# shadygm/Lichtfeld-Densification-Plugin

Measured on AMD Instinct MI355X. Metric: triangulated points/sec + pairs/sec, MipNeRF360 garden @fast, 1/2/4/8 GPU, higher is better.
Workload: dtype f32 (+f64 Sampson/DLT solve)

## Files before the change

lichtfeld-densification-plugin_amd/csrc/lfd_kernels.hip:

```cpp
#include <hip/hip_runtime.h>
#include <stdint.h>

#include "lfd_device.hpp"

namespace {

constexpr int kBlock = LFD_DENSE_BLOCK;
constexpr int kCpt = LFD_DENSE_CPT;
constexpr int kTile = kBlock * kCpt;

typedef unsigned long long u64;

constexpr u64 kStEmpty = 0ull, kStAggregate = 1ull, kStPrefix = 2ull;
constexpr u64 kValueMask = (1ull << LFD_VALUE_BITS) - 1ull;
__device__ __forceinline__ u64 pack_state(u64 st, unsigned epoch, u64 v) {
    return (st << 62) | ((u64)epoch << LFD_VALUE_BITS) | (v & kValueMask);
}
__device__ __forceinline__ u64 state_status(u64 s, unsigned epoch) {
    return (((s >> LFD_VALUE_BITS) & LFD_EPOCH_MASK) == epoch) ? (s >> 62) : kStEmpty;
}

__device__ __forceinline__ void state_store(u64* p, u64 v) {
    __hip_atomic_store(p, v, __ATOMIC_RELAXED, __HIP_MEMORY_SCOPE_AGENT);
}
// ... 178 lines not shown
    if (r >= W) { ++q; r -= W; }
    if (r < 0) { --q; r += W; }
    if (r >= W) { ++q; r -= W; }
    y = q; x = r;
}

__device__ __forceinline__ void lfd_divmod_local(int local, int W, float inv_w, int w_log2, int& dy, int& x) {
    if (w_log2 >= 0) { dy = local >> w_log2; x = local & (W - 1); return; }
    int q = (int)((float)local * inv_w);
    int r = local - __mul24(q, W);
    if (r < 0) { --q; r += W; }
    if (r >= W) { ++q; r -= W; }
    dy = q; x = r;
}

__device__ __forceinline__ float cell_cert(const LfdLaunch& L, const BlockShared& S, int j, int cell, int x, int y,
                                           float raw, float mask_a_val) {
    float c = lfd_cert_floor(raw, L.kp.certainty_thresh);
    if (S.ref.mask_a) c = c * mask_a_val;
    const uint8_t* mb = S.slot[j].mask_b;
    if (mb) {
        const float2 wv = load_f32x2(S.slot[j].warp + (size_t)cell * L.warp_channels + (L.warp_channels - 2));
        const int ix = lfd_grid_nearest(wv.x, L.W);
        const int iy = lfd_grid_nearest(wv.y, L.H);
        float m = 0.0f;
        if (ix >= 0 && iy >= 0)
            m = (float)lfd_global(mb)[(size_t)lfd_nearest_src(iy, L.mask_sy, L.h_match) * L.w_match + lfd_nearest_src(ix, L.mask_sx, L.w_match)];
        c = c * m;
    }
    return c;
}

__device__ __forceinline__ float cell_mask_a(const LfdLaunch& L, const BlockShared& S, int x, int y) {
    if (!S.ref.mask_a) return 1.0f;
    return (float)lfd_global(S.ref.mask_a)[(size_t)lfd_nearest_src(y, L.mask_sy, L.h_match) * L.w_match + lfd_nearest_src(x, L.mask_sx, L.w_match)];
}

__device__ __forceinline__ void argmax_step(float c, int j, float& best, int& bj) {
    const bool take = (c > best) || ((c != c) && !(best != best));
    if (take) { best = c; bj = j; }
}

__device__ __forceinline__ void cell_best(const LfdLaunch& L, const BlockShared& S, int cell, float& best, int& bj) {
    int y, x;
    lfd_divmod(cell, L.W, L.inv_w, y, x);
    const float ma = cell_mask_a(L, S, x, y);
    const int ns = S.ref.n_slots;
    best = cell_cert(L, S, 0, cell, x, y, lfd_global(S.slot[0].cert)[cell], ma);
    bj = 0;
    for (int j = 1; j < ns; ++j) argmax_step(cell_cert(L, S, j, cell, x, y, lfd_global(S.slot[j].cert)[cell], ma), j, best, bj);
}

__device__ __forceinline__ void cells4_best_masked(const LfdLaunch& L, const BlockShared& S, int cell0, int y, int x0,
                                                   float best[4], int bj[4]) {
    const float th = L.kp.certainty_thresh;
    float ma[4] = {1.0f, 1.0f, 1.0f, 1.0f};
    const bool has_a = S.ref.mask_a != nullptr;
    if (has_a) {
        const uint8_t LFD_GLOBAL_AS* row = lfd_global(S.ref.mask_a) + (size_t)lfd_nearest_src(y, L.mask_sy, L.h_match) * L.w_match;
#pragma unroll
        for (int e = 0; e < 4; ++e) ma[e] = (float)row[lfd_nearest_src(x0 + e, L.mask_sx, L.w_match)];
    }
    const int ns = S.ref.n_slots;
    for (int j = 0; j < ns; ++j) {
        const float4 c4 = load_f32x4(S.slot[j].cert + cell0);
        float c[4] = {lfd_cert_floor(c4.x, th), lfd_cert_floor(c4.y, th), lfd_cert_floor(c4.z, th), lfd_cert_floor(c4.w, th)};
        if (has_a) {
#pragma unroll
            for (int e = 0; e < 4; ++e) c[e] = c[e] * ma[e];
        }
        const uint8_t* mb = S.slot[j].mask_b;
        if (mb) {
            float wx[4], wy[4];
            const float* wp = S.slot[j].warp;
            if (L.warp_channels == 4) {
#pragma unroll
                for (int e = 0; e < 4; ++e) { const float4 v = load_f32x4(wp + (size_t)(unsigned)(cell0 + e) * 4); wx[e] = v.z; wy[e] = v.w; }
            } else {
                const float4 a = load_f32x4(wp + (size_t)(unsigned)cell0 * 2), b = load_f32x4(wp + (size_t)(unsigned)cell0 * 2 + 4);
                wx[0] = a.x; wy[0] = a.y; wx[1] = a.z; wy[1] = a.w; wx[2] = b.x; wy[2] = b.y; wx[3] = b.z; wy[3] = b.w;
            }
#pragma unroll
            for (int e = 0; e < 4; ++e) {
                const int ix = lfd_grid_nearest(wx[e], L.W);
                const int iy = lfd_grid_nearest(wy[e], L.H);
                float m = 0.0f;
                if (ix >= 0 && iy >= 0)
                    m = (float)lfd_global(mb)[(size_t)lfd_nearest_src(iy, L.mask_sy, L.h_match) * L.w_match + lfd_nearest_src(ix, L.mask_sx, L.w_match)];
                c[e] = c[e] * m;
            }
        }
        if (j == 0) {
#pragma unroll
            for (int e = 0; e < 4; ++e) { best[e] = c[e]; bj[e] = 0; }
        } else {
#pragma unroll
            for (int e = 0; e < 4; ++e) argmax_step(c[e], j, best[e], bj[e]);
        }
    }
}

__device__ __forceinline__ void cell_coords(const LfdLaunch& L, const BlockShared& S, int cell, int bj, float& xan,
                                            float& yan, float& xbn, float& ybn) {
    const float* wp = S.slot[bj].warp;
    if (L.warp_channels == 4) {
        const float4 v = load_f32x4(wp + (size_t)cell * 4);
        xan = v.x; yan = v.y; xbn = v.z; ybn = v.w;
    } else {
        const float2 v = load_f32x2(wp + (size_t)cell * 2);
        int y, x;
        lfd_divmod(cell, L.W, L.inv_w, y, x);
        xan = lfd_global(L.axis_x)[x]; yan = lfd_global(L.axis_y)[y];
        xbn = v.x; ybn = v.y;
    }
}

}

extern "C" __global__ void lfd_pair_setup_kernel(LfdLaunch L, LfdRefConst* __restrict__ ref_out,
                                                 LfdPairConst* __restrict__ pair_out) {
    const int i = (int)(blockIdx.x * blockDim.x + threadIdx.x);
    const int n_pairs = L.n_refs * L.k;
    if (i < n_pairs) {
        const int r = i / L.k, j = i - r * L.k;
        if (j < L.refs[r].n_slots) {
            lfd_make_pair_const(L.cams[L.refs[r].cam], L.cams[L.slots[i].cam], L.slots[i].cam, L.w_match, L.h_match, pair_out[i],
                                L.fund_override ? L.fund_override + (size_t)i * 9 : nullptr);
        }
    } else if (i < n_pairs + L.n_refs) {
        const int r = i - n_pairs;
        lfd_make_ref_const(L.cams[L.refs[r].cam], L.w_match, L.h_match, ref_out[r]);
    }
}

extern "C" __global__ void __launch_bounds__(256) lfd_aggregate_kernel(LfdLaunch L, float* __restrict__ best_cert,
                                                                       uint8_t* __restrict__ best_slot) {
    __shared__ BlockShared S;
    const int r = (int)blockIdx.y;
    const int tid = (int)threadIdx.x;
    if (tid == 0) S.ref = L.refs[r];
    if (tid < L.k) S.slot[tid] = L.slots[(size_t)r * L.k + tid];
    __syncthreads();
    const int HW = L.H * L.W;
    const bool plain = !S.ref.mask_a && (HW & 3) == 0;
    bool any_mask_b = false;
    for (int j = 0; j < S.ref.n_slots; ++j) any_mask_b |= (S.slot[j].mask_b != nullptr);
    const int ns = S.ref.n_slots;
    for (int base = ((int)blockIdx.x * 256 + tid) * 4; base < HW; base += (int)gridDim.x * 256 * 4) {
        if (plain && !any_mask_b && base + 3 < HW) {
            float4 best = load_f32x4(S.slot[0].cert + base);
            const float th = L.kp.certainty_thresh;
            best.x = lfd_cert_floor(best.x, th); best.y = lfd_cert_floor(best.y, th);
            best.z = lfd_cert_floor(best.z, th); best.w = lfd_cert_floor(best.w, th);
            int b0 = 0, b1 = 0, b2 = 0, b3 = 0;
            for (int j = 1; j < ns; ++j) {
                const float4 c = load_f32x4(S.slot[j].cert + base);
                argmax_step(lfd_cert_floor(c.x, th), j, best.x, b0);
                argmax_step(lfd_cert_floor(c.y, th), j, best.y, b1);
                argmax_step(lfd_cert_floor(c.z, th), j, best.z, b2);
                argmax_step(lfd_cert_floor(c.w, th), j, best.w, b3);
            }
            *reinterpret_cast<float4*>(best_cert + (size_t)r * HW + base) = best;
            if (best_slot) {
                const unsigned packed = (unsigned)b0 | ((unsigned)b1 << 8) | ((unsigned)b2 << 16) | ((unsigned)b3 << 24);
                *reinterpret_cast<unsigned*>(best_slot + (size_t)r * HW + base) = packed;
            }
        } else if ((L.W & 3) == 0 && (HW & 3) == 0 && base + 3 < HW) {
            int y, x0;
            lfd_divmod(base, L.W, L.inv_w, y, x0);
            float b4[4]; int j4[4];
            cells4_best_masked(L, S, base, y, x0, b4, j4);
            *reinterpret_cast<float4*>(best_cert + (size_t)r * HW + base) = make_float4(b4[0], b4[1], b4[2], b4[3]);
            if (best_slot) {
                const unsigned packed = (unsigned)j4[0] | ((unsigned)j4[1] << 8) | ((unsigned)j4[2] << 16) | ((unsigned)j4[3] << 24);
                *reinterpret_cast<unsigned*>(best_slot + (size_t)r * HW + base) = packed;
            }
        } else {
            for (int e = 0; e < 4 && base + e < HW; ++e) {
                float best; int bj;
                cell_best(L, S, base + e, best, bj);
                best_cert[(size_t)r * HW + base + e] = best;
                if (best_slot) best_slot[(size_t)r * HW + base + e] = (uint8_t)bj;
            }
        }
    }
}

#define LFD_CONST_AS __attribute__((address_space(4)))
template <class T>
__device__ __forceinline__ const T LFD_CONST_AS* lfd_const_as(const T* p) {
#pragma clang diagnostic push
#pragma clang diagnostic ignored "-Wold-style-cast"
    return (const T LFD_CONST_AS*)p;
#pragma clang diagnostic pop
}

__device__ __forceinline__ int lfd_slot_bytes12(int sl) {
    int o;
    asm("v_mul_u32_u24 %0, %1, 12" : "=v"(o) : "v"(sl));
    return o;
}

struct DenseStage {
    float xyz[3 * kTile];
    float err[kTile];
    unsigned char slot[kTile];
};

struct __attribute__((packed, aligned(4))) LfdF3 { float a, b, c; };

constexpr int kCopyThreadsOrdered = kBlock - 64;

#if defined(LFD_DENSE_TIMING)
#define LFD_STAMP(i) do { if (L.phase_stamps && lane == 0 && wave < 2) L.phase_stamps[((size_t)blockIdx.x * 2 + wave) * 12 + (i)] = __builtin_readcyclecounter(); } while (0)
#else
#define LFD_STAMP(i) do { } while (0)
#endif

template <bool kExactColour, bool kUnordered = false, bool kPly = false>
__device__ __forceinline__ void lfd_dense_body(const LfdLaunch& L) {
    struct DenseShared {
        BlockShared S;
        DenseStage stage;
        u64 tile_excl;
        unsigned ticket;
        unsigned wave_cnt[kBlock / 64];
        unsigned slot_cnt[LFD_MAX_SLOTS];
    };
    __shared__ DenseShared sh;
    BlockShared& S = sh.S;
    DenseStage& stage = sh.stage;
    static_assert(sizeof(sh.S.pc) >= kTile * sizeof(unsigned short), "the order map does not fit the per-pair constant block");
    unsigned short* const stage_order = reinterpret_cast<unsigned short*>(sh.S.pc);
    unsigned& s_ticket = sh.ticket;
    unsigned (&s_wave_cnt)[kBlock / 64] = sh.wave_cnt;
    unsigned (&s_slot_cnt)[LFD_MAX_SLOTS] = sh.slot_cnt;
    u64& s_tile_excl = sh.tile_excl;

    const int tid = (int)threadIdx.x;
    const int lane = tid & 63, wave = tid >> 6;
#if defined(LFD_DENSE_TIMING)
#endif
    LFD_STAMP(0);
    const unsigned seq = blockIdx.x % LFD_TICKET_LANES;
    const unsigned n_tiles = (unsigned)L.n_refs * (unsigned)L.tiles_per_ref;
    const int HW = L.H * L.W;

#if LFD_STAGGER_UNITS > 0
    if (blockIdx.x < (unsigned)LFD_DENSE_WAVES_PER_SIMD * 256u) {
        const unsigned slot = blockIdx.x >> 8;
        for (unsigned i = 0; i < slot; ++i) __builtin_amdgcn_s_sleep(LFD_STAGGER_UNITS);
    }
#endif
    const unsigned tile_guess = blockIdx.x;
    const int r_guess = __builtin_amdgcn_readfirstlane((int)(tile_guess / (unsigned)L.tiles_per_ref));
#if LFD_FRONT_PRIO > 0
    __builtin_amdgcn_s_setprio(LFD_FRONT_PRIO);
#endif
    PrologueRegs pro;
    if (tile_guess < n_tiles) prologue_issue(L, r_guess, pro);
    if (tid == 0) {
        const unsigned long long k = atomicAdd(L.ticket_lanes + (size_t)seq * 16, 1ull) - L.ticket_base_lane[seq];
        s_ticket = (unsigned)k * LFD_TICKET_LANES + seq;
    }
    if (tid < LFD_MAX_SLOTS) s_slot_cnt[tid] = 0;
    if (tile_guess < n_tiles) prologue_commit(L, pro, S);
    __syncthreads();
    LFD_STAMP(1);
    const unsigned tile = s_ticket;
    if (tile == 0 && (L.seg_counts || kUnordered)) {
        if (L.seg_counts) for (int i = tid; i < L.n_refs * L.k; i += kBlock) L.seg_counts[i] = 0;
        if (kUnordered) for (int i = tid; i < L.n_refs; i += kBlock) L.ref_cursor[i] = 0ull;
        __threadfence();
        __syncthreads();
        if (tid == 0) __hip_atomic_store(L.seg_ready, L.epoch, __ATOMIC_RELEASE, __HIP_MEMORY_SCOPE_AGENT);
    }
    if (tile < n_tiles) {
        const int r = __builtin_amdgcn_readfirstlane((int)(tile / (unsigned)L.tiles_per_ref));
        const int tile_in_ref = (int)(tile - (unsigned)r * (unsigned)L.tiles_per_ref);
        LfdRefConst rc;
        {
            const LfdRefConst LFD_CONST_AS* rcp = lfd_const_as(L.ref_const) + r;
#pragma unroll
            for (int i = 0; i < 12; ++i) rc.P[i] = rcp->P[i];
#pragma unroll
            for (int i = 0; i < 3; ++i) rc.C[i] = rcp->C[i];
            rc.sx = rcp->sx; rc.sy = rcp->sy; rc.pad = 0.0f;
        }
        if (r != r_guess || tile_guess >= n_tiles) {
            __syncthreads();
            block_prologue(L, r, S);
        }
        LFD_STAMP(2);
#if defined(LFD_DENSE_TIMING)
        if (L.phase_stamps && lane == 0 && wave < 2) {
            unsigned long long* s0 = L.phase_stamps + ((size_t)blockIdx.x * 2 + wave) * 12;
            *s0 = (*s0 & ~3ull) | (r == r_guess ? 1ull : 0ull) | (tile == tile_guess ? 2ull : 0ull);
        }
#endif
        const int ns = S.ref.n_slots;
        const bool any_mask = S.ref.any_mask != 0;
        const int tile_cell0 = tile_in_ref * kTile;
        const int cell0 = tile_cell0 + tid * kCpt;
        int tile_y0, tile_x0;
        {
            int ty, tx;
            lfd_divmod(tile_cell0, L.W, L.inv_w, ty, tx);
            tile_y0 = __builtin_amdgcn_readfirstlane(ty); tile_x0 = __builtin_amdgcn_readfirstlane(tx);
        }

        int bj[kCpt];
        unsigned dead = 0;
#if LFD_DENSE_ALL_WARPS
        float spec_xb[4] = {0.0f, 0.0f, 0.0f, 0.0f}, spec_yb[4] = {0.0f, 0.0f, 0.0f, 0.0f};
        bool have_warps = false;
        if (!any_mask && (HW & 3) == 0 && kCpt == 4 && cell0 + 3 < HW && ns <= LFD_DENSE_ALL_WARPS && L.warp_channels == 2) {
            const float th = L.kp.certainty_thresh;
            float4 c[4], wa[4], wb[4];
#pragma unroll
            for (int j = 0; j < 4; ++j) {
                if (j < ns) {
                    c[j] = load_f32x4(S.slot[j].cert + cell0);
                    wa[j] = load_f32x4(S.slot[j].warp + (size_t)(unsigned)cell0 * 2);
                    wb[j] = load_f32x4(S.slot[j].warp + (size_t)(unsigned)cell0 * 2 + 4);
                }
            }
            float4 best = c[0];
            best.x = lfd_cert_floor(best.x, th); best.y = lfd_cert_floor(best.y, th);
            best.z = lfd_cert_floor(best.z, th); best.w = lfd_cert_floor(best.w, th);
            bj[0] = bj[1] = bj[2] = bj[3] = 0;
            spec_xb[0] = wa[0].x; spec_yb[0] = wa[0].y; spec_xb[1] = wa[0].z; spec_yb[1] = wa[0].w;
            spec_xb[2] = wb[0].x; spec_yb[2] = wb[0].y; spec_xb[3] = wb[0].z; spec_yb[3] = wb[0].w;
#pragma unroll
            for (int j = 1; j < 4; ++j) {
                if (j < ns) {
                    int t;
                    t = bj[0]; argmax_step(lfd_cert_floor(c[j].x, th), j, best.x, bj[0]); if (bj[0] != t) { spec_xb[0] = wa[j].x; spec_yb[0] = wa[j].y; }
                    t = bj[1]; argmax_step(lfd_cert_floor(c[j].y, th), j, best.y, bj[1]); if (bj[1] != t) { spec_xb[1] = wa[j].z; spec_yb[1] = wa[j].w; }
                    t = bj[2]; argmax_step(lfd_cert_floor(c[j].z, th), j, best.z, bj[2]); if (bj[2] != t) { spec_xb[2] = wb[j].x; spec_yb[2] = wb[j].y; }
                    t = bj[3]; argmax_step(lfd_cert_floor(c[j].w, th), j, best.w, bj[3]); if (bj[3] != t) { spec_xb[3] = wb[j].z; spec_yb[3] = wb[j].w; }
                }
            }
            have_warps = true;
            if (!(th > 0.0f))
                dead = (unsigned)(best.x <= 0.0f) | ((unsigned)(best.y <= 0.0f) << 1) | ((unsigned)(best.z <= 0.0f) << 2) | ((unsigned)(best.w <= 0.0f) << 3);
        } else
#endif
        if (!any_mask && (HW & 3) == 0 && kCpt == 4 && cell0 + 3 < HW) {
            const float th = L.kp.certainty_thresh;
            float4 best;
            bj[0] = bj[1] = bj[2] = bj[3] = 0;
            {
                best = load_f32x4(S.slot[0].cert + cell0);
                best.x = lfd_cert_floor(best.x, th); best.y = lfd_cert_floor(best.y, th);
                best.z = lfd_cert_floor(best.z, th); best.w = lfd_cert_floor(best.w, th);
                for (int j0 = 1; j0 < ns; j0 += 4) {
                    float4 c[4];
#pragma unroll
                    for (int u = 0; u < 4; ++u)
                        if (j0 + u < ns) c[u] = load_f32x4(S.slot[j0 + u].cert + cell0);
#pragma unroll
                    for (int u = 0; u < 4; ++u) {
                        if (j0 + u < ns) {
                            argmax_step(lfd_cert_floor(c[u].x, th), j0 + u, best.x, bj[0]);
                            argmax_step(lfd_cert_floor(c[u].y, th), j0 + u, best.y, bj[1]);
                            argmax_step(lfd_cert_floor(c[u].z, th), j0 + u, best.z, bj[2]);
                            argmax_step(lfd_cert_floor(c[u].w, th), j0 + u, best.w, bj[3]);
                        }
                    }
                }
            }
            if (!(th > 0.0f))
                dead = (unsigned)(best.x <= 0.0f) | ((unsigned)(best.y <= 0.0f) << 1) | ((unsigned)(best.z <= 0.0f) << 2) | ((unsigned)(best.w <= 0.0f) << 3);
        } else if ((L.W & 3) == 0 && (HW & 3) == 0 && kCpt == 4 && cell0 + 3 < HW) {
            int dy, x0;
            lfd_divmod_local(tile_x0 + tid * kCpt, L.W, L.inv_w, L.w_log2, dy, x0);
            float b4[4];
            cells4_best_masked(L, S, cell0, tile_y0 + dy, x0, b4, bj);
#pragma unroll
            for (int e = 0; e < 4; ++e) dead |= (unsigned)(b4[e] <= 0.0f) << e;
        } else {
#pragma unroll
            for (int e = 0; e < kCpt; ++e) {
                bj[e] = 0;
                if (cell0 + e < HW) { float b; cell_best(L, S, cell0 + e, b, bj[e]); dead |= (unsigned)(b <= 0.0f) << e; }
            }
        }

        LFD_STAMP(3);
        unsigned bj_packed = 0;
#if LFD_WARP_BY_LANE
        const bool wave_whole = kCpt == 4 && (L.W & 3) == 0 && tile_cell0 + (wave + 1) * 64 * kCpt <= HW;
#if LFD_DENSE_ALL_WARPS
        const bool by_lane = wave_whole && !have_warps;
#else
        const bool by_lane = wave_whole;
#endif
        if (by_lane) {
            int t2 = (int)threadIdx.x;
            asm volatile("" : "+v"(t2));
            const int ln = t2 & 63, wv = t2 >> 6;
#pragma unroll
            for (int e = 0; e < 4; ++e) bj_packed |= (unsigned)bj[e] << (8 * e);
            *reinterpret_cast<unsigned*>(&stage.slot[t2 * kCpt]) = bj_packed;
            if (L.warp_channels != 4) {
                int dy, x0;
                lfd_divmod_local(tile_x0 + t2 * kCpt, L.W, L.inv_w, L.w_log2, dy, x0);
                const int y0 = tile_y0 + dy;
                float xa[4], ya;
                if (L.axis_identity) {
#pragma unroll
                    for (int e = 0; e < 4; ++e) xa[e] = lfd_axis_value(L.ax, x0 + e);
                    ya = lfd_axis_value(L.ay, y0);
                } else {
                    const float4 ax = load_f32x4(L.axis_x + x0);
                    xa[0] = ax.x; xa[1] = ax.y; xa[2] = ax.z; xa[3] = ax.w;
                    ya = lfd_global(L.axis_y)[y0];
                }
#pragma unroll
                for (int e = 0; e < 4; ++e) { stage.xyz[3 * (t2 * kCpt + e) + 0] = xa[e]; stage.xyz[3 * (t2 * kCpt + e) + 1] = ya; }
            }
            __builtin_amdgcn_fence(__ATOMIC_ACQ_REL, "wavefront");
            __builtin_amdgcn_wave_barrier();
            const int wbase = wv * 64 * kCpt + ln;
            int sj[4];
#pragma unroll
            for (int e = 0; e < 4; ++e) sj[e] = (int)stage.slot[wbase + 64 * e];
            if (L.warp_channels == 4) {
                float4 v[4];
#pragma unroll
                for (int e = 0; e < 4; ++e) v[e] = load_f32x4(S.slot[sj[e]].warp + (size_t)(unsigned)(tile_cell0 + wbase + 64 * e) * 4);
#pragma unroll
                for (int e = 0; e < 4; ++e) {
                    const int sl = wbase + 64 * e;
                    stage.xyz[3 * sl + 0] = v[e].x; stage.xyz[3 * sl + 1] = v[e].y; stage.xyz[3 * sl + 2] = v[e].z;
                    stage.err[sl] = v[e].w;
                }
            } else {
                float2 v[4];
#pragma unroll
                for (int e = 0; e < 4; ++e) v[e] = load_f32x2(S.slot[sj[e]].warp + (size_t)(unsigned)(tile_cell0 + wbase + 64 * e) * 2);
#pragma unroll
                for (int e = 0; e < 4; ++e) {
                    const int sl = wbase + 64 * e;
                    stage.xyz[3 * sl + 2] = v[e].x;
                    stage.err[sl] = v[e].y;
                }
            }
            __builtin_amdgcn_fence(__ATOMIC_ACQ_REL, "wavefront");
            __builtin_amdgcn_wave_barrier();
        } else
#endif
        if (kCpt == 4 && (L.W & 3) == 0 && cell0 + 3 < HW) {
            float xa[4] = {0.0f, 0.0f, 0.0f, 0.0f}, ya = 0.0f;
            if (L.warp_channels != 4) {
                int dy, x0;
                lfd_divmod_local(tile_x0 + tid * kCpt, L.W, L.inv_w, L.w_log2, dy, x0);
                const int y0 = tile_y0 + dy;
                if (L.axis_identity) {
#pragma unroll
                    for (int e = 0; e < 4; ++e) xa[e] = lfd_axis_value(L.ax, x0 + e);
                    ya = lfd_axis_value(L.ay, y0);
                } else {
                    const float4 ax = load_f32x4(L.axis_x + x0);
                    xa[0] = ax.x; xa[1] = ax.y; xa[2] = ax.z; xa[3] = ax.w;
                    ya = lfd_global(L.axis_y)[y0];
                }
            }
#pragma unroll
            for (int e = 0; e < 4; ++e) {
                const float* wp = S.slot[bj[e]].warp;
                float xan, yan, xbn, ybn;
                if (L.warp_channels == 4) {
                    const float4 v = load_f32x4(wp + (size_t)(unsigned)(cell0 + e) * 4);
                    xan = v.x; yan = v.y; xbn = v.z; ybn = v.w;
#if LFD_DENSE_ALL_WARPS
                } else if (have_warps) {
                    xan = xa[e]; yan = ya; xbn = spec_xb[e]; ybn = spec_yb[e];
#endif
                } else {
                    const float2 v = load_f32x2(wp + (size_t)(unsigned)(cell0 + e) * 2);
                    xan = xa[e]; yan = ya; xbn = v.x; ybn = v.y;
                }
                const int sl = tid * kCpt + e;
                stage.xyz[3 * sl + 0] = xan; stage.xyz[3 * sl + 1] = yan; stage.xyz[3 * sl + 2] = xbn;
                stage.err[sl] = ybn;
                bj_packed |= (unsigned)bj[e] << (8 * e);
            }
        } else {
#pragma unroll
            for (int e = 0; e < kCpt; ++e) {
                float xan = 0.0f, yan = 0.0f, xbn = 0.0f, ybn = 0.0f;
                if (cell0 + e < HW) cell_coords(L, S, cell0 + e, bj[e], xan, yan, xbn, ybn);
                const int sl = tid * kCpt + e;
                stage.xyz[3 * sl + 0] = xan; stage.xyz[3 * sl + 1] = yan; stage.xyz[3 * sl + 2] = xbn;
                stage.err[sl] = ybn;
                bj_packed |= (unsigned)bj[e] << (8 * e);
            }
        }
        if (dead) {
#pragma unroll
            for (int e = 0; e < kCpt; ++e)
                if ((dead >> e) & 1u) stage.xyz[3 * (tid * kCpt + e) + 2] = __builtin_nanf("");
        }
        *reinterpret_cast<unsigned*>(&stage.slot[tid * kCpt]) = bj_packed;

        LFD_STAMP(4);
#if LFD_FRONT_PRIO > 0
        __builtin_amdgcn_s_setprio(0);
#endif
        unsigned keep_bits = 0;
#pragma unroll 1
        for (int ev = 0; ev < kCpt; ++ev) {
            asm volatile("" ::: "memory");
            const int e = __builtin_amdgcn_readfirstlane(ev);
            const int sl = tid * kCpt + e;
            float* sxyz = reinterpret_cast<float*>(reinterpret_cast<unsigned char*>(stage.xyz) + lfd_slot_bytes12(sl));
            const float xan = sxyz[0], yan = sxyz[1], xbn = sxyz[2];
            const float ybn = stage.err[sl];
            const int bje = (int)((bj_packed >> (8 * e)) & 0xffu);
            LfdCellResult res;
            res.keep = 0; res.x = res.y = res.z = res.err = res.xa_px = res.ya_px = 0.0f;
#if defined(LFD_ABLATE_EVAL)
            if (cell0 + e < HW) { res.keep = xbn > -0.9f; res.x = xan; res.y = yan; res.z = xbn; res.err = ybn; res.xa_px = 1.0f; res.ya_px = 1.0f; }
#else
            if (cell0 + e < HW) lfd_eval_correspondence(rc, S.pc[bje], xan, yan, xbn, ybn, L.kp, res);
#endif
            if (res.keep) {
                sxyz[0] = res.x; sxyz[1] = res.y; sxyz[2] = res.z;
                stage.err[sl] = res.err;
                keep_bits |= 1u << e;
            }
        }
        LFD_STAMP(5);
#if defined(LFD_BACK_PRIO)
        __builtin_amdgcn_s_setprio(LFD_BACK_PRIO);
#endif
        if (L.seg_counts) {
            for (int j = 0; j < ns; ++j) {
                unsigned c = 0;
#pragma unroll
                for (int e = 0; e < kCpt; ++e)
                    c += (unsigned)__popcll(__ballot(((keep_bits >> e) & 1u) && ((bj_packed >> (8 * e)) & 0xffu) == (unsigned)j));
                if (lane == 0 && c) atomicAdd(&s_slot_cnt[j], c);
            }
        }

        const unsigned my_cnt = __popc(keep_bits);
        unsigned before = 0, wave_total = 0;
#pragma unroll
        for (int e = 0; e < kCpt; ++e) {
            const u64 m = __ballot((keep_bits >> e) & 1u);
            before += __builtin_amdgcn_mbcnt_hi((unsigned)(m >> 32), __builtin_amdgcn_mbcnt_lo((unsigned)m, 0u));
            wave_total += (unsigned)__popcll(m);
        }
        const unsigned incl = before + my_cnt;
        if (lane == 0) s_wave_cnt[wave] = wave_total;
        __syncthreads();
        LFD_STAMP(6);
        unsigned wave_off = 0, block_total = 0;
#pragma unroll
        for (int w = 0; w < kBlock / 64; ++w) {
            if (w < wave) wave_off += s_wave_cnt[w];
            block_total += s_wave_cnt[w];
        }
        {
            unsigned lpos = wave_off + (incl - my_cnt);
#pragma unroll
            for (int e = 0; e < kCpt; ++e)
                if ((keep_bits >> e) & 1u) stage_order[lpos++] = (unsigned short)(tid * kCpt + e);
        }
        __syncthreads();
        LFD_STAMP(7);
        if (L.seg_counts && tid < ns && s_slot_cnt[tid]) {
            unsigned spins = 0;
            unsigned ready = __hip_atomic_load(L.seg_ready, __ATOMIC_RELAXED, __HIP_MEMORY_SCOPE_AGENT);
            while (ready != L.epoch) {
                if (++spins > LFD_SPIN_LIMIT) { atomicExch(L.status, LFD_LAUNCH_TIMEOUT); break; }
                __builtin_amdgcn_s_sleep(8);
                ready = __hip_atomic_load(L.seg_ready, __ATOMIC_RELAXED, __HIP_MEMORY_SCOPE_AGENT);
            }
            atomicAdd(&L.seg_counts[(size_t)r * L.k + tid], (int)s_slot_cnt[tid]);
        }

        constexpr int kCopyThreads = kUnordered ? kBlock : kCopyThreadsOrdered;
        constexpr int kCopyRecords = (kTile + kCopyThreads - 1) / kCopyThreads;
        float rgb[kCopyRecords][3];
        int ctid = (int)threadIdx.x;
        asm volatile("" : "+v"(ctid));
        if (!kUnordered) ctid -= 64;
        u64 claimed = 0;
        if (kUnordered && tid == 0) {
            unsigned spins = 0;
            unsigned ready = __hip_atomic_load(L.seg_ready, __ATOMIC_RELAXED, __HIP_MEMORY_SCOPE_AGENT);
            while (ready != L.epoch) {
                if (++spins > LFD_SPIN_LIMIT) { atomicExch(L.status, LFD_LAUNCH_TIMEOUT); break; }
                __builtin_amdgcn_s_sleep(8);
                ready = __hip_atomic_load(L.seg_ready, __ATOMIC_RELAXED, __HIP_MEMORY_SCOPE_AGENT);
            }
            claimed = atomicAdd(L.ref_cursor + r, (u64)block_total);
        }
        if (!kUnordered && wave == 0) {
#if defined(LFD_ABLATE_LOOKBACK)
            const u64 excl = (u64)tile * kTile;
#else
            const u64 excl = lookback_exclusive(L, tile, block_total);
#endif
            if (lane == 0) {
                s_tile_excl = excl;
                if (tile_in_ref == 0) L.ref_offsets[r] = (long long)excl;
                if (tile == n_tiles - 1u) L.ref_offsets[L.n_refs] = (long long)(excl + block_total);
            }
        }
        if (kUnordered || wave != 0) {
#if !defined(LFD_ABLATE_STORES)
            const uint8_t* image = S.ref.image;
            const int n_loc = (int)block_total;
            if (!kExactColour && L.colour_cols) {
                const unsigned n_bytes = __umul24((unsigned)L.w_match, (unsigned)L.h_match) * 3u;
#pragma unroll
                for (int u0 = 0; u0 < kCopyRecords; u0 += LFD_COPY_UNROLL) {
                    LfdColourCol cc[LFD_COPY_UNROLL];
                    LfdColourRow cr[LFD_COPY_UNROLL];
                    LfdTapRows taps[LFD_COPY_UNROLL];
                    unsigned sh0[LFD_COPY_UNROLL], sh1[LFD_COPY_UNROLL];
                    if (ctid + u0 * kCopyThreads < n_loc) {
#pragma unroll
                        for (int v = 0; v < LFD_COPY_UNROLL; ++v) {
                            if (u0 + v >= kCopyRecords) break;
                            const int i = ctid + (u0 + v) * kCopyThreads;
                            const int sl = (int)stage_order[i < n_loc ? i : n_loc - 1];
                            int dy, x;
                            lfd_divmod_local(tile_x0 + sl, L.W, L.inv_w, L.w_log2, dy, x);
                            const lfd_u32x4 c4 = *reinterpret_cast<const lfd_u32x4 LFD_GLOBAL_AS*>(lfd_global(L.colour_cols) + x);
                            const lfd_u32x4 r4 = *reinterpret_cast<const lfd_u32x4 LFD_GLOBAL_AS*>(lfd_global(L.colour_rows) + (tile_y0 + dy));
                            cc[v].off = c4.x; cc[v].ax = __uint_as_float(c4.y); cc[v].bx = __uint_as_float(c4.z); cc[v].clamped = c4.w;
                            cr[v].off0 = r4.x; cr[v].off1 = r4.y; cr[v].ay = __uint_as_float(r4.z); cr[v].by = __uint_as_float(r4.w);
                            taps[v] = lfd_bilinear_fetch_tab(image, n_bytes, cc[v], cr[v], sh0[v], sh1[v]);
                        }
#pragma unroll
                        for (int v = 0; v < LFD_COPY_UNROLL; ++v) {
                            if (u0 + v >= kCopyRecords) break;
                            lfd_bilinear_eval_tab(taps[v], sh0[v], sh1[v], cc[v], cr[v], rgb[u0 + v]);
                        }
                    }
                }
            } else {
#pragma unroll
            for (int u0 = 0; u0 < kCopyRecords; u0 += LFD_COPY_UNROLL) {
                float px[LFD_COPY_UNROLL], py[LFD_COPY_UNROLL];
                LfdTapRows taps[LFD_COPY_UNROLL];
                unsigned sh0[LFD_COPY_UNROLL], sh1[LFD_COPY_UNROLL];
                if (ctid + u0 * kCopyThreads < n_loc) {
#pragma unroll
                    for (int v = 0; v < LFD_COPY_UNROLL; ++v) {
                        if (u0 + v >= kCopyRecords) break;
                        const int i = ctid + (u0 + v) * kCopyThreads;
                        const int sl = (int)stage_order[i < n_loc ? i : n_loc - 1];
                        {
                            const int cell = tile_cell0 + sl;
                            float xan, yan;
                            if (L.warp_channels == 4) {
                                const float2 w2 = load_f32x2(S.slot[stage.slot[sl]].warp + (size_t)cell * 4);
                                xan = w2.x; yan = w2.y;
                            } else {
                                int dy, x;
                                lfd_divmod_local(tile_x0 + sl, L.W, L.inv_w, L.w_log2, dy, x);
                                const int y = tile_y0 + dy;
                                if (L.axis_identity) { xan = lfd_axis_value(L.ax, x); yan = lfd_axis_value(L.ay, y); }
                                else { xan = lfd_global(L.axis_x)[x]; yan = lfd_global(L.axis_y)[y]; }
                            }
                            px[v] = lfd_match_px(xan, L.kp.wm1); py[v] = lfd_match_px(yan, L.kp.hm1);
                        }
                        taps[v] = lfd_bilinear_fetch(image, L.w_match, L.h_match, px[v], py[v], sh0[v], sh1[v]);
                    }
#pragma unroll
                    for (int v = 0; v < LFD_COPY_UNROLL; ++v) {
                        if (u0 + v >= kCopyRecords) break;
#if defined(LFD_ABLATE_COLOUR)
                        rgb[u0 + v][0] = px[v]; rgb[u0 + v][1] = py[v]; rgb[u0 + v][2] = (float)(taps[v].r0 + taps[v].r1 + sh0[v] + sh1[v]);
#else
                        if (kExactColour) lfd_bilinear_eval(taps[v], sh0[v], sh1[v], L.w_match, L.h_match, px[v], py[v], rgb[u0 + v]);
                        else lfd_bilinear_eval_f32(taps[v], sh0[v], sh1[v], L.w_match, L.h_match, px[v], py[v], rgb[u0 + v]);
#endif
                    }
                }
            }
            }
#endif
        }
        if (kUnordered && tid == 0) {
            s_tile_excl = (u64)(unsigned)r * (u64)(unsigned)HW + claimed;
            LfdTileSeg seg; seg.offset = (int32_t)claimed; seg.count = (int32_t)block_total;
            L.tile_table[tile] = seg;
        }
        LFD_STAMP(8);
        __syncthreads();
        LFD_STAMP(9);

#if !defined(LFD_ABLATE_STORES)
        if (kUnordered || wave != 0) {
            const u64 excl = s_tile_excl;
            const long long base = (long long)(((u64)(unsigned)__builtin_amdgcn_readfirstlane((int)(unsigned)(excl >> 32)) << 32) |
                                               (u64)(unsigned)__builtin_amdgcn_readfirstlane((int)(unsigned)excl));
            long long room = L.capacity - base;
            int n = (int)block_total;
            if (room < (long long)n) n = room > 0 ? (int)room : 0;
            if (kPly) {
                unsigned char* gp = L.ply + 15 * base;
#pragma unroll
                for (int u = 0; u < kCopyRecords; ++u) {
                    const int i = ctid + u * kCopyThreads;
                    if (i < n) {
                        const int sl = (int)stage_order[i];
                        const float* sxyz = reinterpret_cast<const float*>(reinterpret_cast<const unsigned char*>(stage.xyz) + lfd_slot_bytes12(sl));
                        struct __attribute__((packed, aligned(1))) F3u { float a, b, c; };
                        struct __attribute__((packed, aligned(1))) U16u { unsigned short v; };
                        F3u p; p.a = sxyz[0]; p.b = sxyz[1]; p.c = sxyz[2];
                        const unsigned o15 = (unsigned)i * 15u;
                        const unsigned q0 = lfd_quantise_u8(rgb[u][0]), q1 = lfd_quantise_u8(rgb[u][1]), q2 = lfd_quantise_u8(rgb[u][2]);
                        *reinterpret_cast<F3u*>(gp + o15) = p;
                        U16u rg; rg.v = (unsigned short)(q0 | (q1 << 8));
                        *reinterpret_cast<U16u*>(gp + o15 + 12u) = rg;
                        gp[o15 + 14u] = (unsigned char)q2;
                        if (L.cell) L.cell[base + i] = tile_cell0 + sl;
                        if (L.slot) L.slot[base + i] = stage.slot[sl];
                    }
                }
            } else {
            unsigned char* gx = reinterpret_cast<unsigned char*>(L.xyz + 3 * base);
            unsigned char* gc = reinterpret_cast<unsigned char*>(L.rgb + 3 * base);
            unsigned char* ge = reinterpret_cast<unsigned char*>(L.err + base);
#pragma unroll
            for (int u = 0; u < kCopyRecords; ++u) {
                const int i = ctid + u * kCopyThreads;
                if (i < n) {
                    const int sl = (int)stage_order[i];
                    LfdF3 p, c;
                    const float* sxyz = reinterpret_cast<const float*>(reinterpret_cast<const unsigned char*>(stage.xyz) + lfd_slot_bytes12(sl));
                    p.a = sxyz[0]; p.b = sxyz[1]; p.c = sxyz[2];
                    c.a = rgb[u][0]; c.b = rgb[u][1]; c.c = rgb[u][2];
                    const unsigned o12 = (unsigned)lfd_slot_bytes12(i), o4 = (unsigned)i * 4u;
#if LFD_NT_STORES
                    float* fx = reinterpret_cast<float*>(gx + o12);
                    float* fc = reinterpret_cast<float*>(gc + o12);
                    __builtin_nontemporal_store(p.a, fx); __builtin_nontemporal_store(p.b, fx + 1); __builtin_nontemporal_store(p.c, fx + 2);
                    __builtin_nontemporal_store(c.a, fc); __builtin_nontemporal_store(c.b, fc + 1); __builtin_nontemporal_store(c.c, fc + 2);
                    __builtin_nontemporal_store(stage.err[sl], reinterpret_cast<float*>(ge + o4));
#else
                    *reinterpret_cast<LfdF3*>(gx + o12) = p;
                    *reinterpret_cast<LfdF3*>(gc + o12) = c;
                    *reinterpret_cast<float*>(ge + o4) = stage.err[sl];
#endif
                    if (L.cell) L.cell[base + i] = tile_cell0 + sl;
                    if (L.slot) L.slot[base + i] = stage.slot[sl];
                }
            }
        }
#endif
            }
#if defined(LFD_DENSE_TIMING)
        LFD_STAMP(10);
        if (L.phase_stamps && lane == 0 && wave < 2) {
            asm volatile("s_waitcnt vmcnt(0)" ::: "memory");
            L.phase_stamps[((size_t)blockIdx.x * 2 + wave) * 12 + 11] = __builtin_readcyclecounter();
        }
#endif
    }
}

extern "C" __global__ void __launch_bounds__(kBlock, LFD_DENSE_WAVES_PER_SIMD) lfd_dense_kernel(LfdLaunch L) { lfd_dense_body<false>(L); }
extern "C" __global__ void __launch_bounds__(kBlock, LFD_DENSE_WAVES_PER_SIMD) lfd_dense_exact_kernel(LfdLaunch L) { lfd_dense_body<true>(L); }
extern "C" __global__ void __launch_bounds__(kBlock, LFD_DENSE_WAVES_PER_SIMD) lfd_dense_ply_kernel(LfdLaunch L) { lfd_dense_body<false, false, true>(L); }
extern "C" __global__ void __launch_bounds__(kBlock, LFD_DENSE_WAVES_PER_SIMD) lfd_dense_ply_exact_kernel(LfdLaunch L) { lfd_dense_body<true, false, true>(L); }
extern "C" __global__ void __launch_bounds__(kBlock, LFD_DENSE_WAVES_PER_SIMD) lfd_dense_segments_kernel(LfdLaunch L) { lfd_dense_body<false, true>(L); }
extern "C" __global__ void __launch_bounds__(kBlock, LFD_DENSE_WAVES_PER_SIMD) lfd_dense_segments_exact_kernel(LfdLaunch L) { lfd_dense_body<true, true>(L); }
extern "C" __global__ void __launch_bounds__(kBlock, LFD_DENSE_WAVES_PER_SIMD) lfd_dense_ply_segments_kernel(LfdLaunch L) { lfd_dense_body<false, true, true>(L); }
extern "C" __global__ void __launch_bounds__(kBlock, LFD_DENSE_WAVES_PER_SIMD) lfd_dense_ply_segments_exact_kernel(LfdLaunch L) { lfd_dense_body<true, true, true>(L); }

extern "C" __global__ void __launch_bounds__(LFD_INDEXED_EVAL_BLOCK) lfd_indexed_eval_kernel(LfdLaunch L, const long long* __restrict__ sel_idx,
                                                                                             const long long* __restrict__ sel_offsets,
                                                                                             float* __restrict__ scratch, uint8_t* __restrict__ codes,
                                                                                             unsigned* __restrict__ tab, int off_pairs) {
    __shared__ BlockShared S;
    __shared__ unsigned s_cnt[LFD_MAX_SLOTS];
    __shared__ unsigned s_first[LFD_MAX_SLOTS];
    const int tid = (int)threadIdx.x;
    const int r = (int)blockIdx.y;
    const long long sel_begin = off_pairs ? sel_offsets[2 * r] : sel_offsets[r], sel_end = off_pairs ? sel_offsets[2 * r + 1] : sel_offsets[r + 1];
    const int n_sel = (int)(sel_end - sel_begin);
    const int i = (int)blockIdx.x * LFD_INDEXED_EVAL_BLOCK + tid;
    if ((int)blockIdx.x * LFD_INDEXED_EVAL_BLOCK >= n_sel) return;
    if (tid < LFD_MAX_SLOTS) { s_cnt[tid] = 0; s_first[tid] = 0xffffffffu; }
    block_prologue(L, r, S);
    const int HW = L.H * L.W;
    if (i < n_sel) {
        const long long cl = sel_idx[sel_begin + i];
        unsigned code = 0xffu;
        if (cl >= 0 && cl < HW) {
            const int cell = (int)cl;
            float best; int bj;
            cell_best(L, S, cell, best, bj);
            float xan, yan, xbn, ybn;
            cell_coords(L, S, cell, bj, xan, yan, xbn, ybn);
            LfdCellResult res;
            lfd_eval_correspondence(S.rc, S.pc[bj], xan, yan, xbn, ybn, L.kp, res);
            atomicMin(&s_first[bj], (unsigned)i);
            code = (unsigned)bj | (res.keep ? 0x80u : 0u);
            if (res.keep) {
                float rgb[3];
                lfd_bilinear_rgb(S.ref.image, L.w_match, L.h_match, res.xa_px, res.ya_px, 1.0f, 1.0f, rgb);
                float* o = scratch + (size_t)(sel_begin + i) * 8;
                o[0] = res.x; o[1] = res.y; o[2] = res.z; o[3] = res.err; o[4] = rgb[0]; o[5] = rgb[1]; o[6] = rgb[2];
                atomicAdd(&s_cnt[bj], 1u);
            }
        }
        codes[sel_begin + i] = (uint8_t)code;
    }
    __syncthreads();
    if (tid < LFD_MAX_SLOTS) {
        unsigned* t = tab + ((size_t)r * LFD_MAX_SLOTS + tid) * 2;
        if (s_cnt[tid]) atomicAdd(t + 0, s_cnt[tid]);
        if (s_first[tid] != 0xffffffffu) atomicMax(t + 1, 0xffffffffu - s_first[tid]);
    }
}

extern "C" __global__ void __launch_bounds__(LFD_INDEXED_BLOCK) lfd_indexed_kernel(LfdLaunch L, const long long* __restrict__ sel_idx,
                                                                                   const long long* __restrict__ sel_offsets,
                                                                                   float* __restrict__ scratch, uint8_t* __restrict__ codes,
                                                                                   int32_t* __restrict__ seg_order, const unsigned* __restrict__ tab, int off_pairs) {
    __shared__ BlockShared S;
    __shared__ unsigned s_ticket;
    __shared__ unsigned s_cnt[LFD_MAX_SLOTS];
    __shared__ unsigned s_first[LFD_MAX_SLOTS];
    __shared__ unsigned s_start[LFD_MAX_SLOTS];
    __shared__ unsigned s_run[LFD_MAX_SLOTS];
    __shared__ unsigned s_wcnt[LFD_INDEXED_BLOCK / 64][LFD_MAX_SLOTS];
    __shared__ u64 s_excl;
    __shared__ unsigned s_total;

    const int tid = (int)threadIdx.x, lane = tid & 63, wave = tid >> 6;
    constexpr int nwaves = LFD_INDEXED_BLOCK / 64;
    if (tid == 0) s_ticket = (unsigned)(atomicAdd(L.ticket, 1ull) - L.ticket_base);
    if (tid < LFD_MAX_SLOTS) { s_cnt[tid] = 0; s_first[tid] = 0xffffffffu; s_run[tid] = 0; }
    __syncthreads();
    const int r = (int)s_ticket;
    block_prologue(L, r, S);
    const int ns = S.ref.n_slots;
    const long long sel_begin = off_pairs ? sel_offsets[2 * r] : sel_offsets[r], sel_end = off_pairs ? sel_offsets[2 * r + 1] : sel_offsets[r + 1];
    const int n_sel = (int)(sel_end - sel_begin);
    const int HW = L.H * L.W;

    if (tab) {
        if (tid < LFD_MAX_SLOTS) {
            s_cnt[tid] = tab[((size_t)r * LFD_MAX_SLOTS + tid) * 2 + 0];
            s_first[tid] = 0xffffffffu - tab[((size_t)r * LFD_MAX_SLOTS + tid) * 2 + 1];
        }
    }
    for (int i = tid; i < (tab ? 0 : n_sel); i += LFD_INDEXED_BLOCK) {
        const long long cl = sel_idx[sel_begin + i];
        unsigned code = 0xffu;
        if (cl >= 0 && cl < HW) {
            const int cell = (int)cl;
            float best; int bj;
            cell_best(L, S, cell, best, bj);
            float xan, yan, xbn, ybn;
            cell_coords(L, S, cell, bj, xan, yan, xbn, ybn);
            LfdCellResult res;
            lfd_eval_correspondence(S.rc, S.pc[bj], xan, yan, xbn, ybn, L.kp, res);
            atomicMin(&s_first[bj], (unsigned)i);
// ... 79 lines not shown
```

Measured before the change: 51.88 billion.

## Evaluate by-lane staged cells contiguously per wave step and fold keep bits into slots

When the by-lane staging path runs, each lane in the per-cell evaluation loop now reads cells strided by 64 within its wave's segment, using the slot indices already loaded per lane, instead of four consecutive cells per thread. Each wave step therefore covers adjacent pixels, which are more likely to share a neighbour slot and a similar solver iteration count, so divergence in lfd_eval_correspondence should drop. Keep flags are packed into the top bit of each slot byte to save registers, and the compaction order is rebuilt with per-step ballots so output order stays consistent. This adds index arithmetic and requires at most 128 slots. Profiling scripts for A/B timing and slot uniformity are also added.

New measurement: 52.43 billion (median of 4 runs). +1.1%, better.

```diff
diff --git a/lichtfeld-densification-plugin_amd/csrc/lfd_kernels.hip b/lichtfeld-densification-plugin_amd/csrc/lfd_kernels.hip
--- a/lichtfeld-densification-plugin_amd/csrc/lfd_kernels.hip
+++ b/lichtfeld-densification-plugin_amd/csrc/lfd_kernels.hip
@@ -504,6 +504,7 @@
         const bool any_mask = S.ref.any_mask != 0;
         const int tile_cell0 = tile_in_ref * kTile;
         const int cell0 = tile_cell0 + tid * kCpt;
+        const int wave_u = __builtin_amdgcn_readfirstlane(wave);
         int tile_y0, tile_x0;
         {
             int ty, tx;
@@ -591,8 +592,9 @@
 
         LFD_STAMP(3);
         unsigned bj_packed = 0;
+        bool contig = false;
 #if LFD_WARP_BY_LANE
-        const bool wave_whole = kCpt == 4 && (L.W & 3) == 0 && tile_cell0 + (wave + 1) * 64 * kCpt <= HW;
+        const bool wave_whole = kCpt == 4 && (L.W & 3) == 0 && tile_cell0 + (wave_u + 1) * 64 * kCpt <= HW;
 #if LFD_DENSE_ALL_WARPS
         const bool by_lane = wave_whole && !have_warps;
 #else
@@ -651,6 +653,10 @@
             }
             __builtin_amdgcn_fence(__ATOMIC_ACQ_REL, "wavefront");
             __builtin_amdgcn_wave_barrier();
+            bj_packed = 0;
+#pragma unroll
+            for (int e = 0; e < 4; ++e) bj_packed |= (unsigned)sj[e] << (8 * e);
+            contig = true;
         } else
 #endif
         if (kCpt == 4 && (L.W & 3) == 0 && cell0 + 3 < HW) {
@@ -705,35 +711,41 @@
             for (int e = 0; e < kCpt; ++e)
                 if ((dead >> e) & 1u) stage.xyz[3 * (tid * kCpt + e) + 2] = __builtin_nanf("");
         }
-        *reinterpret_cast<unsigned*>(&stage.slot[tid * kCpt]) = bj_packed;
+        if (!contig) *reinterpret_cast<unsigned*>(&stage.slot[tid * kCpt]) = bj_packed;
 
         LFD_STAMP(4);
 #if LFD_FRONT_PRIO > 0
         __builtin_amdgcn_s_setprio(0);
 #endif
-        unsigned keep_bits = 0;
+        static_assert(LFD_MAX_SLOTS <= 128, "the top bit of a slot byte is taken");
+        const int contig_s = __builtin_amdgcn_readfirstlane(contig ? 1 : 0);
+        const int sl_off0 = contig_s * wave_u * (64 * (kCpt - 1));
 #pragma unroll 1
         for (int ev = 0; ev < kCpt; ++ev) {
             asm volatile("" ::: "memory");
             const int e = __builtin_amdgcn_readfirstlane(ev);
-            const int sl = tid * kCpt + e;
+            int cg = contig_s;
+            asm volatile("" : "+s"(cg));
+            const int sl = ((tid * kCpt) >> (2 * cg)) + (sl_off0 + e * (1 + 63 * cg));
             float* sxyz = reinterpret_cast<float*>(reinterpret_cast<unsigned char*>(stage.xyz) + lfd_slot_bytes12(sl));
             const float xan = sxyz[0], yan = sxyz[1], xbn = sxyz[2];
             const float ybn = stage.err[sl];
-            const int bje = (int)((bj_packed >> (8 * e)) & 0xffu);
+            const int bje = (int)((bj_packed >> (8 * e)) & 0x7fu);
             LfdCellResult res;
             res.keep = 0; res.x = res.y = res.z = res.err = res.xa_px = res.ya_px = 0.0f;
 #if defined(LFD_ABLATE_EVAL)
-            if (cell0 + e < HW) { res.keep = xbn > -0.9f; res.x = xan; res.y = yan; res.z = xbn; res.err = ybn; res.xa_px = 1.0f; res.ya_px = 1.0f; }
+            if (tile_cell0 + sl < HW) { res.keep = xbn > -0.9f; res.x = xan; res.y = yan; res.z = xbn; res.err = ybn; res.xa_px = 1.0f; res.ya_px = 1.0f; }
 #else
-            if (cell0 + e < HW) lfd_eval_correspondence(rc, S.pc[bje], xan, yan, xbn, ybn, L.kp, res);
+            if (tile_cell0 + sl < HW) lfd_eval_correspondence(rc, S.pc[bje], xan, yan, xbn, ybn, L.kp, res);
 #endif
             if (res.keep) {
                 sxyz[0] = res.x; sxyz[1] = res.y; sxyz[2] = res.z;
                 stage.err[sl] = res.err;
-                keep_bits |= 1u << e;
-            }
-        }
+                bj_packed |= 0x80u << (8 * e);
+            }
+        }
+        const unsigned keep_bits = ((bj_packed >> 7) & 1u) | ((bj_packed >> 14) & 2u) | ((bj_packed >> 21) & 4u) | ((bj_packed >> 28) & 8u);
+        bj_packed &= 0x7f7f7f7fu;
         LFD_STAMP(5);
 #if defined(LFD_BACK_PRIO)
         __builtin_amdgcn_s_setprio(LFD_BACK_PRIO);
@@ -748,7 +760,6 @@
             }
         }
 
-        const unsigned my_cnt = __popc(keep_bits);
         unsigned before = 0, wave_total = 0;
 #pragma unroll
         for (int e = 0; e < kCpt; ++e) {
@@ -756,7 +767,6 @@
             before += __builtin_amdgcn_mbcnt_hi((unsigned)(m >> 32), __builtin_amdgcn_mbcnt_lo((unsigned)m, 0u));
             wave_total += (unsigned)__popcll(m);
         }
-        const unsigned incl = before + my_cnt;
         if (lane == 0) s_wave_cnt[wave] = wave_total;
         __syncthreads();
         LFD_STAMP(6);
@@ -766,8 +776,17 @@
             if (w < wave) wave_off += s_wave_cnt[w];
             block_total += s_wave_cnt[w];
         }
-        {
-            unsigned lpos = wave_off + (incl - my_cnt);
+        if (contig_s) {
+            unsigned run = wave_off;
+#pragma unroll
+            for (int e = 0; e < kCpt; ++e) {
+                const u64 m = __ballot((keep_bits >> e) & 1u);
+                const unsigned below = __builtin_amdgcn_mbcnt_hi((unsigned)(m >> 32), __builtin_amdgcn_mbcnt_lo((unsigned)m, 0u));
+                if ((keep_bits >> e) & 1u) stage_order[run + below] = (unsigned short)(((tid * kCpt) >> 2) + wave_u * (64 * (kCpt - 1)) + 64 * e);
+                run += (unsigned)__popcll(m);
+            }
+        } else {
+            unsigned lpos = wave_off + before;
 #pragma unroll
             for (int e = 0; e < kCpt; ++e)
                 if ((keep_bits >> e) & 1u) stage_order[lpos++] = (unsigned short)(tid * kCpt + e);
diff --git a/profiles/ab_scalar_pair.py b/profiles/ab_scalar_pair.py
--- /dev/null
+++ b/profiles/ab_scalar_pair.py
@@ -0,0 +1,53 @@
+#!/usr/bin/env python3
+import argparse
+import json
+import os
+import subprocess
+import sys
+
+import numpy as np
+
+ROOT = os.path.dirname(os.path.dirname(os.path.abspath(__file__)))
+
+
+def main():
+    ap = argparse.ArgumentParser()
+    ap.add_argument("--parent", required=True, help="liblfd_densify.so built from the parent commit")
+    ap.add_argument("--new", default=os.path.join(ROOT, "lichtfeld-densification-plugin_amd", "liblfd_densify.so"))
+    ap.add_argument("--also", action="append", default=[], metavar="NAME=PATH", help="a further library to time")
+    ap.add_argument("--passes", type=int, default=3)
+    ap.add_argument("--steps", type=int, default=3000)
+    ap.add_argument("--limit-s", type=float, default=150.0, help="time limit of one bench process")
+    args, extra = ap.parse_known_args()
+    variants = [("parent", args.parent), ("new", args.new)] + [tuple(a.split("=", 1)) for a in args.also]
+    res = {name: {"kernel_ms": [], "ms_per_step": []} for name, _ in variants}
+    for p in range(args.passes):
+        for name, lib in variants:
+            env = dict(os.environ, LFD_DENSIFY_LIB=lib)
+            cmd = [sys.executable, os.path.join(ROOT, "bench.py"), "--gpus", "1", "--light", "--cpu-sample-refs", "0", "--parity-refs", "0",
+                   "--steps", str(args.steps)] + extra
+            try:
+                out = subprocess.run(cmd, env=env, capture_output=True, text=True, timeout=args.limit_s)
+            except subprocess.TimeoutExpired:
+                raise SystemExit(f"pass {p} {name}: no result within {args.limit_s} s - stopping")
+            line = [l for l in out.stdout.splitlines() if l.startswith("{")]
+            if out.returncode != 0 or not line:
+                raise SystemExit(f"pass {p} {name}: FAILED (exit {out.returncode}) {out.stderr[-600:]} - stopping")
+            d = json.loads(line[0])
+            res[name]["kernel_ms"].append(d["roofline"]["kernel_ms"])
+            res[name]["ms_per_step"].append(d["ms_per_step"])
+            print(f"pass {p} {name:16s} kernel_ms {d['roofline']['kernel_ms']:.4f}  ms_per_step {d['ms_per_step']:.4f}  surv {d['survivor_fraction']:.6f}", flush=True)
+    for key in ("kernel_ms", "ms_per_step"):
+        base = res["parent"][key]
+        spread = float(np.max(base) - np.min(base))
+        print(f"-- {key}: parent spread (max - min over {len(base)} passes) {spread:.4f} ms = {spread / np.mean(base):.2%}")
+        for name, _ in variants:
+            v = res[name][key]
+            m = float(np.mean(v))
+            d = m - float(np.mean(base))
+            print(f"{name:16s} mean {m:.4f} ms  sd {np.std(v):.4f}  spread {np.max(v) - np.min(v):.4f}  {d / np.mean(base):+.2%} vs parent"
+                  + (f"  = {d / spread:+.1f} parent spreads" if spread > 0 and name != "parent" else ""))
+
+
+if __name__ == "__main__":
+    main()
diff --git a/profiles/slot_uniformity.py b/profiles/slot_uniformity.py
--- /dev/null
+++ b/profiles/slot_uniformity.py
@@ -0,0 +1,54 @@
+#!/usr/bin/env python3
+import os
+import sys
+
+import numpy as np
+
+ROOT = os.path.dirname(os.path.dirname(os.path.abspath(__file__)))
+sys.path.insert(0, ROOT)
+sys.path.insert(0, os.path.dirname(os.path.abspath(__file__)))
+from lichtfeld_densification_plugin_amd import synthetic
+from solver_stats import build_rows, solves_needed
+
+
+def by_step(per_cell, mapping):
+    v = per_cell.reshape(-1, 4, 256)
+    if mapping == "strided":
+        return v.reshape(-1, 4, 64, 4).transpose(0, 1, 3, 2)
+    return v.reshape(-1, 4, 4, 64)
+
+
+def main():
+    n_refs = int(sys.argv[1]) if len(sys.argv) > 1 else 2
+    H = W = wm = hm = 512
+    cams = synthetic.ring_cameras(185, seed=0)
+    for k in (3, 8):
+        for gi in range(n_refs):
+            ref = (gi * 3) % 185
+            nbrs = synthetic.ring_neighbours(185, ref, k)
+            s = synthetic.synth_reference(cams, ref, nbrs, H, W, wm, hm, noise_px=0.5, outlier_frac=0.05, channels=2, seed=1000 + gi,
+                                          cert_mode="smooth")
+            cert = np.maximum(s.cert.numpy(), np.float32(0.2))
+            bj = cert.argmax(0)
+            Aw = np.empty((H, W, 4, 4), np.float32)
+            se = np.empty((H, W))
+            for j in range(k):
+                A, sj = build_rows(cams, s, j, H, W, wm, hm)
+                m = bj == j
+                Aw[m] = A[m]; se[m] = sj[m]
+            passed = (se < 5.0).reshape(-1)
+            it = np.zeros(H * W, int)
+            idx = np.nonzero(passed)[0]
+            it[idx] = solves_needed(Aw.reshape(-1, 4, 4)[idx])[0]
+            for mapping in ("strided", "consecutive"):
+                slots = by_step(bj.reshape(-1), mapping)
+                uniform = (slots == slots[..., :1]).all(axis=-1)
+                itw = by_step(it, mapping)
+                wave_max = itw.max(axis=-1)
+                active = wave_max > 0
+                print(f"k={k} ref {gi} {mapping:11s}: wave steps with one slot {uniform.mean():.3f}; distinct slots per step {np.mean([len(np.unique(r)) for r in slots.reshape(-1, 64)]):.2f}; "
+                      f"solves per wave step {wave_max[active].mean():.2f} (cells {it[idx].mean():.2f})")
+
+
+if __name__ == "__main__":
+    main()
```
